# mims-harvard/Raindrop

Measured on AMD Instinct MI355X. Metric: samples/sec fwd+bwd, P19 34-sensor batch=256; % HBM roofline on msg-pass kernel, higher is better.
Workload: dtype f32

## Files before the change

### raindrop_amd/csrc/rd_attnfuse.hip

```cpp
#include <stdlib.h>

#include "rd_common.h"
#include "rd_plan.h"
#include "rd_rng.h"

namespace rd {
namespace {

typedef __bf16 bf8 __attribute__((ext_vector_type(8)));
typedef __bf16 bf4 __attribute__((ext_vector_type(4)));
typedef short sh4 __attribute__((ext_vector_type(4)));
typedef short sh8 __attribute__((ext_vector_type(8)));

constexpr int TS = 64;
constexpr int LDT = TS;
__device__ __forceinline__ int tsw(int row) { return (row & 3) | (((row >> 3) & 1) << 2); }
__device__ __forceinline__ int tofs(int row, int col) { return row * LDT + ((((col >> 3) ^ tsw(row)) & 7) << 3) + (col & 7); }
constexpr int AF_WV = 8, AF_THR = 64 * AF_WV;

struct FAttnArgs {
  const float* x;
  const __bf16* wf;
  const __bf16* wb;
  const float* bias;
  float* out; float* lse;
  const float* dout; const float* ds1; float* dx;
  __bf16* xt; __bf16* dt;
  const int32_t* plan;
  int T, B, D, H, hd;
  float scale, p_drop; uint64_t seed; uint32_t site; const uint64_t* seed_cell;
  int one;
  unsigned long long* stamps;
};
static unsigned long long* g_af_stamps = nullptr;
#define AFSTAMP(i)                                                                                  \
  do {                                                                                              \
    if (a.stamps && blockIdx.x == 0 && threadIdx.x == 0) a.stamps[(i)] = clock64();                 \
  } while (0)

__device__ __forceinline__ float g16_max(float v) {
#define RD_ROR(v, n) __builtin_bit_cast(float, __builtin_amdgcn_update_dpp(0, __builtin_bit_cast(int, v), 0x120 + (n), 0xf, 0xf, false))
  v = fmaxf(v, RD_ROR(v, 8)); v = fmaxf(v, RD_ROR(v, 4)); v = fmaxf(v, RD_ROR(v, 2)); v = fmaxf(v, RD_ROR(v, 1));
  return v;
}
__device__ __forceinline__ float g16_sum(float v) {
  v += RD_ROR(v, 8); v += RD_ROR(v, 4); v += RD_ROR(v, 2); v += RD_ROR(v, 1);
#undef RD_ROR
  return v;
}

__device__ __forceinline__ bf8 frag_n(const __bf16* P, int ld, int row0, int k0, int lane) {
  return *reinterpret_cast<const bf8*>(P + (row0 + (lane & 15)) * ld + k0 + 8 * (lane >> 4));
}
__device__ __forceinline__ bf8 frag_t(const __bf16* P, int ld, int k0, int col0, int lane) {
  const int i = lane & 15, G = lane >> 4;
  const __bf16* src = P + (k0 + 8 * G + (i >> 2)) * ld + col0 + 4 * (i & 3);
  const sh4 lo = __builtin_amdgcn_ds_read_tr16_b64_v4i16((sh4 __attribute__((address_space(3)))*)(src));
  const sh4 hi = __builtin_amdgcn_ds_read_tr16_b64_v4i16((sh4 __attribute__((address_space(3)))*)(src + 4 * ld));
  const sh8 o = {lo[0], lo[1], lo[2], lo[3], hi[0], hi[1], hi[2], hi[3]};
  return __builtin_bit_cast(bf8, o);
}
__device__ __forceinline__ bf8 frag_ns(const __bf16* P, int row0, int k0, int lane) {
  return *reinterpret_cast<const bf8*>(P + tofs(row0 + (lane & 15), k0 + 8 * (lane >> 4)));
}
__device__ __forceinline__ bf8 frag_ts(const __bf16* P, int k0, int col0, int lane) {
  const int i = lane & 15, G = lane >> 4;
  const int row = k0 + 8 * G + (i >> 2), col = col0 + 4 * (i & 3);
  const __bf16* src = P + tofs(row, col);
  const sh4 lo = __builtin_amdgcn_ds_read_tr16_b64_v4i16((sh4 __attribute__((address_space(3)))*)(src));
  const sh4 hi = __builtin_amdgcn_ds_read_tr16_b64_v4i16((sh4 __attribute__((address_space(3)))*)(src + 4 * LDT));
  const sh8 o = {lo[0], lo[1], lo[2], lo[3], hi[0], hi[1], hi[2], hi[3]};
  return __builtin_bit_cast(bf8, o);
}
template <int NT, bool AT, bool BT, bool ASW, bool BSW>
__device__ __forceinline__ void mma_b16(f32x4 (&acc)[NT], const __bf16* Ah, const __bf16* Al, int lda, int a0, const __bf16* Bh,
                                        const __bf16* Bl, int ldb, int b0, int KK, int lane, bool one) {
  auto fa = [&](const __bf16* P, int k0) {
    if (ASW) return AT ? frag_ts(P, k0, a0, lane) : frag_ns(P, a0, k0, lane);
    return AT ? frag_t(P, lda, k0, a0, lane) : frag_n(P, lda, a0, k0, lane);
  };
  auto fb = [&](const __bf16* P, int k0, int j) {
    if (BSW) return BT ? frag_ts(P, k0, b0 + 16 * j, lane) : frag_ns(P, b0 + 16 * j, k0, lane);
    return BT ? frag_t(P, ldb, k0, b0 + 16 * j, lane) : frag_n(P, ldb, b0 + 16 * j, k0, lane);
  };
  if (!one) {
#pragma unroll
    for (int k0 = 0; k0 < KK; k0 += 32) {
      const bf8 ah = fa(Ah, k0);
      const bf8 al = fa(Al, k0);
      bf8 bh[NT], bl[NT];
#pragma unroll
      for (int j = 0; j < NT; ++j) { bh[j] = fb(Bh, k0, j); bl[j] = fb(Bl, k0, j); }
#pragma unroll
      for (int j = 0; j < NT; ++j) acc[j] = __builtin_amdgcn_mfma_f32_16x16x32_bf16(al, bh[j], acc[j], 0, 0, 0);
#pragma unroll
      for (int j = 0; j < NT; ++j) acc[j] = __builtin_amdgcn_mfma_f32_16x16x32_bf16(ah, bl[j], acc[j], 0, 0, 0);
#pragma unroll
      for (int j = 0; j < NT; ++j) acc[j] = __builtin_amdgcn_mfma_f32_16x16x32_bf16(ah, bh[j], acc[j], 0, 0, 0);
    }
  } else {
#pragma unroll
    for (int k0 = 0; k0 < KK; k0 += 32) {
      const bf8 ah = fa(Ah, k0);
#pragma unroll
      for (int j = 0; j < NT; ++j) {
        const bf8 bh = fb(Bh, k0, j);
        acc[j] = __builtin_amdgcn_mfma_f32_16x16x32_bf16(ah, bh, acc[j], 0, 0, 0);
      }
    }
  }
}

__device__ __forceinline__ void split4(const float (&v)[4], bf4& hi, bf4& lo) {
#pragma unroll
  for (int r = 0; r < 4; ++r) { hi[r] = (__bf16)v[r]; lo[r] = (__bf16)(v[r] - (float)hi[r]); }
}
__device__ __forceinline__ void store_t4(__bf16* Ph, __bf16* Pl, int row, int col4, const float (&v)[4]) {
  bf4 hi, lo;
  split4(v, hi, lo);
  const int o = tofs(row, col4);
  *reinterpret_cast<bf4*>(Ph + o) = hi;
  *reinterpret_cast<bf4*>(Pl + o) = lo;
}

__device__ __forceinline__ uint64_t attn_quad(int bh, int T, int q, int key) { return ((uint64_t)bh * T + key) * ((T + 3) >> 2) + (q >> 2); }
__device__ __forceinline__ void attn_keep4(float (&k4)[4], uint64_t seed, uint32_t site, int bh, int T, int q0, int key, float p, float inv_keep) {
  const float4 u = uniform4(seed, site, attn_quad(bh, T, q0, key));
  k4[0] = u.x >= p ? inv_keep : 0.f; k4[1] = u.y >= p ? inv_keep : 0.f;
  k4[2] = u.z >= p ? inv_keep : 0.f; k4[3] = u.w >= p ? inv_keep : 0.f;
}

template <int KCX>
struct XRows { float4 v[(TS * 8 * KCX) / AF_THR]; };

template <int KCX>
__device__ __forceinline__ void x_request(XRows<KCX>& r, const float* x, long row0, int Tv, int D, int tid) {
  constexpr int kq = 8 * KCX, NIT = (TS * kq) / AF_THR;
  static_assert((TS * kq) % AF_THR == 0, "x tile must divide over the workgroup");
#pragma unroll
  for (int it = 0; it < NIT; ++it) {
    const int i = tid + it * AF_THR;
    const int rr = i / kq, k = 4 * (i - rr * kq);
    r.v[it] = *reinterpret_cast<const float4*>(x + (row0 + min(rr, Tv - 1)) * D + min(k, D - 4));
  }
}
template <int KCX>
__device__ __forceinline__ void x_store(const XRows<KCX>& r, __bf16* Xh, __bf16* Xl, int Tv, int D, int tid) {
  constexpr int kq = 8 * KCX, NIT = (TS * kq) / AF_THR, LDX = 32 * KCX + 16;
#pragma unroll
  for (int it = 0; it < NIT; ++it) {
    const int i = tid + it * AF_THR;
    const int rr = i / kq, k = 4 * (i - rr * kq);
    const bool ok = rr < Tv && k < D;
    const float v[4] = {ok ? r.v[it].x : 0.f, ok ? r.v[it].y : 0.f, ok ? r.v[it].z : 0.f, ok ? r.v[it].w : 0.f};
    bf4 hi, lo;
    split4(v, hi, lo);
    *reinterpret_cast<bf4*>(Xh + rr * LDX + k) = hi;
    *reinterpret_cast<bf4*>(Xl + rr * LDX + k) = lo;
  }
}

template <int KCX>
struct QkvPanel { bf8 h[2][KCX], l[2][KCX]; float bs[2]; };

template <int NTH, int KCX>
__device__ __forceinline__ void qkv_request(QkvPanel<KCX>& p, const __bf16* wf_h, const float* bias, int D, int hd, int h, int wave, int lane) {
  constexpr int NCT3 = 3 * NTH;
  static_assert(NCT3 <= 2 * AF_WV, "two column tiles per wave");
#pragma unroll
  for (int s = 0; s < 2; ++s) {
    const int ct = min(wave + AF_WV * s, NCT3 - 1);
    const __bf16* t = wf_h + (size_t)ct * (KCX * 2 * 512) + lane * 8;
#pragma unroll
    for (int kc = 0; kc < KCX; ++kc) {
      p.h[s][kc] = *reinterpret_cast<const bf8*>(t + (kc * 2 + 0) * 512);
      p.l[s][kc] = *reinterpret_cast<const bf8*>(t + (kc * 2 + 1) * 512);
    }
    const int whc = ct / NTH, cl = 16 * (ct - whc * NTH) + (lane & 15);
    p.bs[s] = bias[whc * D + h * hd + min(cl, hd - 1)];
  }
}

template <int NTH, int KCX>
__device__ __forceinline__ void qkv_project(const QkvPanel<KCX>& p, const __bf16* Xh, const __bf16* Xl, int hd, int Tv, __bf16* Tp, int wave,
                                            int lane, bool one) {
  constexpr int NCT3 = 3 * NTH, HDP = 32 * ((16 * NTH + 31) / 32), LDX = 32 * KCX + 16;
  const bool two = wave + AF_WV < NCT3;
  const int aoff = (lane & 15) * LDX + 8 * (lane >> 4);
  f32x4 acc[2][4];
#pragma unroll
  for (int s = 0; s < 2; ++s)
#pragma unroll
    for (int rt = 0; rt < 4; ++rt) acc[s][rt] = (f32x4){0.f, 0.f, 0.f, 0.f};
  if (!one) {
#pragma unroll
    for (int kc = 0; kc < KCX; ++kc) {
      bf8 ah[4], al[4];
#pragma unroll
      for (int rt = 0; rt < 4; ++rt) {
        ah[rt] = *reinterpret_cast<const bf8*>(Xh + rt * 16 * LDX + aoff + kc * 32);
        al[rt] = *reinterpret_cast<const bf8*>(Xl + rt * 16 * LDX + aoff + kc * 32);
      }
#pragma unroll
      for (int s = 0; s < 2; ++s)
#pragma unroll
        for (int rt = 0; rt < 4; ++rt) acc[s][rt] = __builtin_amdgcn_mfma_f32_16x16x32_bf16(al[rt], p.h[s][kc], acc[s][rt], 0, 0, 0);
#pragma unroll
      for (int s = 0; s < 2; ++s)
#pragma unroll
        for (int rt = 0; rt < 4; ++rt) acc[s][rt] = __builtin_amdgcn_mfma_f32_16x16x32_bf16(ah[rt], p.l[s][kc], acc[s][rt], 0, 0, 0);
#pragma unroll
      for (int s = 0; s < 2; ++s)
#pragma unroll
        for (int rt = 0; rt < 4; ++rt) acc[s][rt] = __builtin_amdgcn_mfma_f32_16x16x32_bf16(ah[rt], p.h[s][kc], acc[s][rt], 0, 0, 0);
    }
  } else {
#pragma unroll
    for (int kc = 0; kc < KCX; ++kc) {
#pragma unroll
      for (int rt = 0; rt < 4; ++rt) {
        const bf8 ah = *reinterpret_cast<const bf8*>(Xh + rt * 16 * LDX + aoff + kc * 32);
#pragma unroll
        for (int s = 0; s < 2; ++s) acc[s][rt] = __builtin_amdgcn_mfma_f32_16x16x32_bf16(ah, p.h[s][kc], acc[s][rt], 0, 0, 0);
      }
    }
  }
#pragma unroll
  for (int s = 0; s < 2; ++s) {
    if (s == 1 && !two) break;
    const int ct = wave + AF_WV * s;
    const int whc = ct / NTH, cl = 16 * (ct - whc * NTH) + (lane & 15);
    __bf16* Ph = Tp + (size_t)(whc * 2) * HDP * LDT;
    __bf16* Pl = Ph + (size_t)HDP * LDT;
    const bool cok = cl < hd;
#pragma unroll
    for (int rt = 0; rt < 4; ++rt) {
      const int r0 = 16 * rt + 4 * (lane >> 4);
      float v[4];
#pragma unroll
      for (int r = 0; r < 4; ++r) v[r] = (cok && r0 + r < Tv) ? acc[s][rt][r] + p.bs[s] : 0.f;
      store_t4(Ph, Pl, cl, r0, v);
    }
  }
}

template <int NTH>
__device__ __forceinline__ void zero_pad_rows(__bf16* Tp, int tid) {
  constexpr int HDP = 32 * ((16 * NTH + 31) / 32), PADR = HDP - 16 * NTH;
  if (PADR == 0) return;
  constexpr int Q8 = LDT / 4;
  for (int i = tid; i < 6 * PADR * Q8; i += AF_THR) {
    const int pl = i / (PADR * Q8), rem = i - pl * (PADR * Q8);
    const int rr = rem / Q8, q = rem - rr * Q8;
    bf4 z;
#pragma unroll
    for (int c = 0; c < 4; ++c) z[c] = (__bf16)0.f;
    *reinterpret_cast<bf4*>(Tp + ((size_t)pl * HDP + 16 * NTH + rr) * LDT + 4 * q) = z;
  }
}

template <int NTH, int KCX, bool ONE>
__global__ __launch_bounds__(AF_THR) void k_attn_fwd_fused(FAttnArgs a) {
  extern __shared__ __attribute__((aligned(16))) unsigned char fsm[];
  RD_TOUCH_CODE(ONE ? RD_TL_ATTN_FWD_B : RD_TL_ATTN_FWD);
  constexpr int HDP = 32 * ((16 * NTH + 31) / 32), LDX = 32 * KCX + 16, NA = (NTH + 1) / 2;
  constexpr int LDO = 16 * NTH + 4;
  __bf16* Xh = reinterpret_cast<__bf16*>(fsm);
  __bf16* Xl = Xh + TS * LDX;
  __bf16* Tp = Xl + TS * LDX;
  __bf16 *Qh = Tp, *Ql = Qh + HDP * LDT, *Kh = Ql + HDP * LDT, *Kl = Kh + HDP * LDT, *Vh = Kl + HDP * LDT, *Vl = Vh + HDP * LDT;
  float* mxs = reinterpret_cast<float*>(Vl + HDP * LDT);
  float* sms = mxs + 2 * TS;
  __bf16 *Ph = Qh, *Pl = Ql;
  float* ost = reinterpret_cast<float*>(Kh);
  static_assert(HDP >= TS, "P^T must fit inside the Q^T plane");
  static_assert((size_t)TS * LDO * 4 <= (size_t)2 * HDP * LDT * 2, "output stage must fit inside the K^T planes");
  const int tid = threadIdx.x, lane = tid & 63, wave = __builtin_amdgcn_readfirstlane(tid >> 6), wq = wave & 3, wh = wave >> 2;
  const int b = blockIdx.x;
  const int Tv = __builtin_amdgcn_readfirstlane(a.plan[plan::len_base(a.B) + b]);
  if (Tv <= 0) return;
  const long row0 = __builtin_amdgcn_readfirstlane(a.plan[plan::off_base() + b]);
  uint64_t seedv = a.seed;
  XRows<KCX> xr;
  x_request<KCX>(xr, a.x, row0, Tv, a.D, tid);
  QkvPanel<KCX> pan;
  qkv_request<NTH, KCX>(pan, a.wf, a.bias, a.D, a.hd, 0, wave, lane);
  __builtin_amdgcn_sched_barrier(0);
  if (a.p_drop > 0.f && a.seed_cell) seedv += load_uniform_u64(a.seed_cell);
  zero_pad_rows<NTH>(Tp, tid);
  AFSTAMP(0);
  x_store<KCX>(xr, Xh, Xl, Tv, a.D, tid);
  AFSTAMP(1);
  lds_barrier();
  AFSTAMP(2);
  const float inv_keep = 1.0f / (1.0f - a.p_drop);
  constexpr bool one = ONE;
  const int qr0 = wq * 16 + 4 * (lane >> 4);
  for (int h = 0; h < a.H; ++h) {
    const int bh = b * a.H + h;
    if (h > 0) zero_pad_rows<NTH>(Tp, tid);
    qkv_project<NTH, KCX>(pan, Xh, Xl, a.hd, Tv, Tp, wave, lane, one);
    __builtin_amdgcn_sched_barrier(0);
    {
      const int hn = h + 1 < a.H ? h + 1 : 0;
      qkv_request<NTH, KCX>(pan, a.wf + (size_t)hn * (3 * NTH * KCX * 2 * 512), a.bias, a.D, a.hd, hn, wave, lane);
    }
    __builtin_amdgcn_sched_barrier(0);
    AFSTAMP(3 + 8 * h);
    lds_barrier();
    AFSTAMP(4 + 8 * h);
    float kp[2][4];
#pragma unroll
    for (int j = 0; j < 2; ++j)
      attn_keep4(kp[j], seedv, a.site, bh, a.T, qr0, min(16 * (2 * wh + j) + (lane & 15), a.T - 1), a.p_drop, inv_keep);
    f32x4 s[2];
#pragma unroll
    for (int j = 0; j < 2; ++j) s[j] = (f32x4){0.f, 0.f, 0.f, 0.f};
    mma_b16<2, true, true, true, true>(s, Qh, Ql, LDT, wq * 16, Kh, Kl, LDT, 32 * wh, HDP, lane, one);
    float mx[4] = {-INFINITY, -INFINITY, -INFINITY, -INFINITY};
#pragma unroll
    for (int j = 0; j < 2; ++j) {
      const int key = 16 * (2 * wh + j) + (lane & 15);
      const bool dead = key >= Tv;
#pragma unroll
      for (int r = 0; r < 4; ++r) {
        s[j][r] = dead ? -INFINITY : s[j][r] * a.scale;
        mx[r] = fmaxf(mx[r], s[j][r]);
      }
    }
#pragma unroll
    for (int r = 0; r < 4; ++r) {
      mx[r] = g16_max(mx[r]);
      if ((lane & 15) == 0) mxs[wh * TS + qr0 + r] = mx[r];
    }
    AFSTAMP(5 + 8 * h);
    lds_barrier();
    float m_i[4], rsum[4] = {0.f, 0.f, 0.f, 0.f};
#pragma unroll
    for (int r = 0; r < 4; ++r) m_i[r] = fmaxf(mxs[qr0 + r], mxs[TS + qr0 + r]);
#pragma unroll
    for (int j = 0; j < 2; ++j) {
      const int key = 16 * (2 * wh + j) + (lane & 15);
      float pv[4];
#pragma unroll
      for (int r = 0; r < 4; ++r) {
        const float p = (s[j][r] == -INFINITY) ? 0.f : __expf(s[j][r] - m_i[r]);
        rsum[r] += p;
        pv[r] = p * kp[j][r];
      }
      store_t4(Ph, Pl, key, qr0, pv);
    }
#pragma unroll
    for (int r = 0; r < 4; ++r) {
      rsum[r] = g16_sum(rsum[r]);
      if ((lane & 15) == 0) sms[wh * TS + qr0 + r] = rsum[r];
    }
    AFSTAMP(6 + 8 * h);
    lds_barrier();
    AFSTAMP(7 + 8 * h);
    float l_i[4];
#pragma unroll
    for (int r = 0; r < 4; ++r) l_i[r] = sms[qr0 + r] + sms[TS + qr0 + r];
    const int t0 = wh * NA;
    f32x4 o[NA];
#pragma unroll
    for (int j = 0; j < NA; ++j) o[j] = (f32x4){0.f, 0.f, 0.f, 0.f};
    mma_b16<NA, true, false, true, true>(o, Ph, Pl, LDT, wq * 16, Vh, Vl, LDT, 16 * t0, TS, lane, one);
#pragma unroll
    for (int r = 0; r < 4; ++r) {
      const int q = qr0 + r;
      const float inv = 1.0f / l_i[r];
#pragma unroll
      for (int j = 0; j < NA; ++j)
        if (t0 + j < NTH) ost[q * LDO + 16 * (t0 + j) + (lane & 15)] = o[j][r] * inv;
      if (wh == 0 && (lane & 15) == 0 && q < Tv) a.lse[(long)bh * a.T + q] = m_i[r] + logf(l_i[r]);
    }
    AFSTAMP(8 + 8 * h);
    lds_barrier();
    AFSTAMP(9 + 8 * h);
    {
      const int qpr = a.hd >> 2;
      for (int e = tid; e < Tv * qpr; e += AF_THR) {
        const int q = e / qpr, c4 = e - q * qpr;
        *reinterpret_cast<float4*>(a.out + (row0 + q) * a.D + h * a.hd + 4 * c4) = *reinterpret_cast<const float4*>(ost + q * LDO + 4 * c4);
      }
    }
    lds_barrier();
    AFSTAMP(10 + 8 * h);
  }
}

template <int NTH, int KCX>
constexpr size_t fwd_lds() {
  constexpr int HDP = 32 * ((16 * NTH + 31) / 32), LDX = 32 * KCX + 16;
  return (size_t)2 * TS * LDX * 2 + (size_t)6 * HDP * LDT * 2 + (size_t)4 * TS * 4;
}

template <int NTH>
struct HRegs { float4 v[(4 * NTH + 7) / 8]; unsigned ok; };
template <int NTH>
__device__ __forceinline__ void head_request(HRegs<NTH>& h, const float* base, long ld, int Tv, int hd, int tl) {
  constexpr int NCH = (4 * NTH + 7) / 8;
  const int t = tl >> 3;
  const bool rok = t < Tv;
  const float* src = base + (long)(rok ? t : 0) * ld;
  unsigned ok = 0;
#pragma unroll
  for (int i = 0; i < NCH; ++i) {
    const int c = 4 * ((tl & 7) + 8 * i);
    const bool cok = c < hd;
    h.v[i] = *reinterpret_cast<const float4*>(src + (cok ? c : 0));
    if (rok && cok) ok |= 1u << i;
  }
  h.ok = ok;
}
template <int NTH>
__device__ __forceinline__ void head_mask(HRegs<NTH>& h) {
  constexpr int NCH = (4 * NTH + 7) / 8;
#pragma unroll
  for (int i = 0; i < NCH; ++i)
    if (!((h.ok >> i) & 1u)) h.v[i] = make_float4(0.f, 0.f, 0.f, 0.f);
}

template <int KB>
struct DxPanel { bf8 h[2][KB], l[2][KB]; };

template <int KCX, int KB, int NS>
__device__ __forceinline__ void dx_request(DxPanel<KB>& p, const __bf16* wb_h, int which, int wave, int lane) {
  constexpr int NCT = 2 * KCX;
#pragma unroll
  for (int s = 0; s < NS; ++s) {
    const __bf16* t = wb_h + ((size_t)which * NCT + wave + AF_WV * s) * (KB * 2 * 512) + lane * 8;
#pragma unroll
    for (int kc = 0; kc < KB; ++kc) {
      p.h[s][kc] = *reinterpret_cast<const bf8*>(t + (kc * 2 + 0) * 512);
      p.l[s][kc] = *reinterpret_cast<const bf8*>(t + (kc * 2 + 1) * 512);
    }
  }
}
template <int NTH, int KB, int NS, bool ONE>
__device__ __forceinline__ void dx_mma(f32x4 (&dxa)[2][4], const DxPanel<KB>& p, const __bf16* Tp, int which, int lane) {
  constexpr int HDP = 32 * ((16 * NTH + 31) / 32);
  const __bf16* Ah = Tp + (size_t)(which * 2) * HDP * LDT;
  const __bf16* Al = Ah + (size_t)HDP * LDT;
#pragma unroll
  for (int kc = 0; kc < KB; ++kc) {
    bf8 ah[4], al[4];
#pragma unroll
    for (int rt = 0; rt < 4; ++rt) {
      ah[rt] = frag_ts(Ah, 32 * kc, 16 * rt, lane);
      if (!ONE) al[rt] = frag_ts(Al, 32 * kc, 16 * rt, lane);
    }
    if (!ONE) {
#pragma unroll
      for (int s = 0; s < NS; ++s)
#pragma unroll
        for (int rt = 0; rt < 4; ++rt) dxa[s][rt] = __builtin_amdgcn_mfma_f32_16x16x32_bf16(al[rt], p.h[s][kc], dxa[s][rt], 0, 0, 0);
#pragma unroll
      for (int s = 0; s < NS; ++s)
#pragma unroll
        for (int rt = 0; rt < 4; ++rt) dxa[s][rt] = __builtin_amdgcn_mfma_f32_16x16x32_bf16(ah[rt], p.l[s][kc], dxa[s][rt], 0, 0, 0);
    }
#pragma unroll
    for (int s = 0; s < NS; ++s)
#pragma unroll
      for (int rt = 0; rt < 4; ++rt) dxa[s][rt] = __builtin_amdgcn_mfma_f32_16x16x32_bf16(ah[rt], p.h[s][kc], dxa[s][rt], 0, 0, 0);
  }
}
template <int NTH, int KCX, int NS, bool ONE>
__device__ __forceinline__ void dx_phase(f32x4 (&dxa)[2][4], DxPanel<(16 * NTH + 31) / 32>& p0, const __bf16* Tp, const __bf16* wb_h, int wave,
                                         int lane) {
  constexpr int KB = (16 * NTH + 31) / 32;
  DxPanel<KB> p1;
  dx_request<KCX, KB, NS>(p1, wb_h, 1, wave, lane);
  __builtin_amdgcn_sched_barrier(0);
  dx_mma<NTH, KB, NS, ONE>(dxa, p0, Tp, 0, lane);
  __builtin_amdgcn_sched_barrier(0);
  dx_request<KCX, KB, NS>(p0, wb_h, 2, wave, lane);
  __builtin_amdgcn_sched_barrier(0);
  dx_mma<NTH, KB, NS, ONE>(dxa, p1, Tp, 1, lane);
  __builtin_amdgcn_sched_barrier(0);
  dx_mma<NTH, KB, NS, ONE>(dxa, p0, Tp, 2, lane);
  __builtin_amdgcn_sched_barrier(0);
}

template <int NTH, int KCX, bool ONE>
__global__ __launch_bounds__(AF_THR) void k_attn_bwd_fused(FAttnArgs a) {
  extern __shared__ __attribute__((aligned(16))) unsigned char fsm[];
  RD_TOUCH_CODE(ONE ? RD_TL_ATTN_BWD_B : RD_TL_ATTN_BWD);
  constexpr int HDP = 32 * ((16 * NTH + 31) / 32), LDX = 32 * KCX + 16, NA = (NTH + 1) / 2, KB = HDP / 32, LDB = HDP + 16;
  constexpr int NCT = 2 * KCX;
  constexpr int LDS_DX = 32 * KCX + 4;
  __bf16* Xh = reinterpret_cast<__bf16*>(fsm);
  __bf16* Xl = Xh + TS * LDX;
  __bf16 *Ph = Xh, *Pl = Ph + TS * LDT, *Sh = Pl + TS * LDT, *Sl = Sh + TS * LDT;
  float* dxs = reinterpret_cast<float*>(fsm);
  static_assert((size_t)4 * TS * LDT * 2 <= (size_t)2 * TS * LDX * 2, "score planes must fit inside the x planes");
  static_assert((size_t)TS * LDS_DX * 4 <= (size_t)2 * TS * LDX * 2, "dx stage must fit inside the x planes");
  __bf16* Tp = Xl + TS * LDX;
  __bf16 *Qh = Tp, *Ql = Qh + HDP * LDT, *Kh = Ql + HDP * LDT, *Kl = Kh + HDP * LDT, *Vh = Kl + HDP * LDT, *Vl = Vh + HDP * LDT;
  __bf16* Oh = Vl + HDP * LDT;
  __bf16* Ol = Oh + TS * LDB;
  float* lse_s = reinterpret_cast<float*>(Ol + TS * LDB);
  float* dl_s = lse_s + TS;
  const int tid = threadIdx.x, lane = tid & 63, wave = __builtin_amdgcn_readfirstlane(tid >> 6), wq = wave & 3, wh = wave >> 2;
  const int b = blockIdx.x;
  const int Tv = __builtin_amdgcn_readfirstlane(a.plan[plan::len_base(a.B) + b]);
  if (Tv <= 0) return;
  const long row0 = __builtin_amdgcn_readfirstlane(a.plan[plan::off_base() + b]);
  const int g0 = __builtin_amdgcn_readfirstlane(a.plan[plan::coff_base(a.B, a.T) + b]);
  const int ngrp = (Tv + 15) >> 4;
  const bool tail_zero = (g0 + ngrp) == __builtin_amdgcn_readfirstlane(a.plan[plan::coff_base(a.B, a.T) + a.B]) && ((g0 + ngrp) & 1);
  uint64_t seedv = a.seed;
  if (a.p_drop > 0.f && a.seed_cell) seedv += load_uniform_u64(a.seed_cell);
  const float inv_keep = 1.0f / (1.0f - a.p_drop);
  constexpr bool one = ONE;
  f32x4 dxa[2][4];
#pragma unroll
  for (int s = 0; s < 2; ++s)
#pragma unroll
    for (int rt = 0; rt < 4; ++rt) dxa[s][rt] = (f32x4){0.f, 0.f, 0.f, 0.f};
  const bool two = wave + AF_WV < NCT;
  constexpr int NQ = (TS * 8 * KCX + AF_THR - 1) / AF_THR;
  QkvPanel<KCX> pan;
  HRegs<NTH> dov, ov; float lrow;
  head_request<NTH>(dov, a.dout + row0 * a.D, a.D, Tv, a.hd, tid);
  head_request<NTH>(ov, a.out + row0 * a.D, a.D, Tv, a.hd, tid);
  lrow = a.lse[(long)(b * a.H) * a.T + min(tid >> 3, Tv - 1)];
  for (int h = 0; h < a.H; ++h) {
    const int bh = b * a.H + h;
    int tl = tid;
    asm volatile("" : "+v"(tl));
    XRows<KCX> xr;
    x_request<KCX>(xr, a.x, row0, Tv, a.D, tl);
    int lq = lane;
    asm volatile("" : "+v"(lq));
    qkv_request<NTH, KCX>(pan, a.wf + (size_t)h * (3 * NTH * KCX * 2 * 512), a.bias, a.D, a.hd, h, wave, lq);
    AFSTAMP(32 + 16 * h);
    __builtin_amdgcn_sched_barrier(0);
    if (h == 0) zero_pad_rows<NTH>(Tp, tl);
    x_store<KCX>(xr, Xh, Xl, Tv, a.D, tl);
    AFSTAMP(33 + 16 * h);
    lds_barrier();
    AFSTAMP(34 + 16 * h);
    if (h == 0) {
      const int i16 = lq & 15, g2 = (lq >> 4) & 1, sub = lq >> 5;
      const int npair = (ngrp + 1) >> 1;
      for (int t = wave; t < npair * NCT * 2; t += AF_WV) {
        const int plane = t & 1, cj = t >> 1;
        const int pr = cj / NCT, j = cj - pr * NCT;
        const int lg = 2 * pr + sub;
        const __bf16* src = (plane ? Xl : Xh) + (16 * min(lg, ngrp - 1) + 8 * g2 + (i16 >> 2)) * LDX + 16 * j + 4 * (i16 & 3);
        const sh4 lo = __builtin_amdgcn_ds_read_tr16_b64_v4i16((sh4 __attribute__((address_space(3)))*)(src));
        const sh4 hi = __builtin_amdgcn_ds_read_tr16_b64_v4i16((sh4 __attribute__((address_space(3)))*)(src + 4 * LDX));
        const sh8 o = {lo[0], lo[1], lo[2], lo[3], hi[0], hi[1], hi[2], hi[3]};
        const int gg = g0 + lg;
        if (lg < ngrp)
          *reinterpret_cast<sh8*>(a.xt + (((size_t)(gg >> 1) * NCT + j) * 2 + plane) * 512 + (32 * (gg & 1) + 16 * g2 + i16) * 8) = o;
      }
      if (tail_zero) {
        const int gg = g0 + ngrp;
        const sh8 z = {0, 0, 0, 0, 0, 0, 0, 0};
        for (int i = tid; i < NCT * 2 * 32; i += AF_THR) {
          const int slot = i & 31, jp = i >> 5;
          *reinterpret_cast<sh8*>(a.xt + ((size_t)(gg >> 1) * NCT * 2 + jp) * 512 + (32 + slot) * 8) = z;
        }
      }
    }
    {
      constexpr int NCH = (4 * NTH + 7) / 8;
      head_mask<NTH>(dov);
      head_mask<NTH>(ov);
      float d = 0.f;
#pragma unroll
      for (int i = 0; i < NCH; ++i)
        d += (dov.v[i].x * ov.v[i].x + dov.v[i].y * ov.v[i].y) + (dov.v[i].z * ov.v[i].z + dov.v[i].w * ov.v[i].w);
      d += __shfl_xor(d, 1);
      d += __shfl_xor(d, 2);
      d += __shfl_xor(d, 4);
      const int o = (tl >> 3) * LDB + 4 * (tl & 7);
#pragma unroll
      for (int i = 0; i < NCH; ++i) {
        static_assert(32 * NCH == HDP, "8 threads x NCH chunks cover exactly the padded head width (chunks >= hd arrive as zeros)");
        const float v[4] = {dov.v[i].x, dov.v[i].y, dov.v[i].z, dov.v[i].w};
        bf4 hi, lo;
        split4(v, hi, lo);
        *reinterpret_cast<bf4*>(Oh + o + 32 * i) = hi;
        *reinterpret_cast<bf4*>(Ol + o + 32 * i) = lo;
      }
      if ((tl & 7) == 0) { dl_s[tl >> 3] = d; lse_s[tl >> 3] = lrow; }
    }
    __builtin_amdgcn_sched_barrier(0);
    {
      const int hn = h + 1 < a.H ? h + 1 : 0;
      head_request<NTH>(dov, a.dout + row0 * a.D + hn * a.hd, a.D, Tv, a.hd, tl);
      head_request<NTH>(ov, a.out + row0 * a.D + hn * a.hd, a.D, Tv, a.hd, tl);
      lrow = a.lse[(long)(b * a.H + hn) * a.T + min(tl >> 3, Tv - 1)];
    }
    AFSTAMP(35 + 16 * h);
    __builtin_amdgcn_sched_barrier(0);
    qkv_project<NTH, KCX>(pan, Xh, Xl, a.hd, Tv, Tp, wave, lq, one);
    AFSTAMP(36 + 16 * h);
    lds_barrier();
    AFSTAMP(37 + 16 * h);
    int l1 = lane;
    asm volatile("" : "+v"(l1));
    const int qr1 = wq * 16 + 4 * (l1 >> 4);
    float kp[2][4];
#pragma unroll
    for (int j = 0; j < 2; ++j)
      attn_keep4(kp[j], seedv, a.site, bh, a.T, qr1, min(16 * (2 * wh + j) + (l1 & 15), a.T - 1), a.p_drop, inv_keep);
    f32x4 s[2], dp[2];
#pragma unroll
    for (int j = 0; j < 2; ++j) { s[j] = (f32x4){0.f, 0.f, 0.f, 0.f}; dp[j] = s[j]; }
    mma_b16<2, true, true, true, true>(s, Qh, Ql, LDT, wq * 16, Kh, Kl, LDT, 32 * wh, HDP, l1, one);
    mma_b16<2, false, true, false, true>(dp, Oh, Ol, LDB, wq * 16, Vh, Vl, LDT, 32 * wh, HDP, l1, one);
#pragma unroll
    for (int j = 0; j < 2; ++j) {
      const int key = 16 * (2 * wh + j) + (l1 & 15);
      const bool dead = key >= Tv;
      const float (&k4)[4] = kp[j];
      float pm[4], ds[4];
#pragma unroll
      for (int r = 0; r < 4; ++r) {
        const int row = qr1 + r;
        pm[r] = 0.f; ds[r] = 0.f;
        if (!dead && row < Tv) {
          const float p = __expf(s[j][r] * a.scale - lse_s[row]);
          pm[r] = p * k4[r];
          ds[r] = p * (dp[j][r] * k4[r] - dl_s[row]) * a.scale;
        }
      }
      store_t4(Ph, Pl, key, qr1, pm);
      store_t4(Sh, Sl, key, qr1, ds);
    }
    AFSTAMP(38 + 16 * h);
    lds_barrier();
    AFSTAMP(39 + 16 * h);
    const int t0 = wh * NA;
    int l2 = lane;
    asm volatile("" : "+v"(l2));
    f32x4 dq[NA], dk[NA], dv[NA];
#pragma unroll
    for (int j = 0; j < NA; ++j) { dq[j] = (f32x4){0.f, 0.f, 0.f, 0.f}; dk[j] = dq[j]; dv[j] = dq[j]; }
    mma_b16<NA, true, false, true, true>(dq, Sh, Sl, LDT, wq * 16, Kh, Kl, LDT, 16 * t0, TS, l2, one);
    mma_b16<NA, false, false, true, true>(dk, Sh, Sl, LDT, wq * 16, Qh, Ql, LDT, 16 * t0, TS, l2, one);
    mma_b16<NA, false, true, true, false>(dv, Ph, Pl, LDT, wq * 16, Oh, Ol, LDB, 16 * t0, TS, l2, one);
    AFSTAMP(40 + 16 * h);
    lds_barrier();
    AFSTAMP(41 + 16 * h);
    const __bf16* wb_h = a.wb + (size_t)h * (3 * NCT * KB * 2 * 512);
    DxPanel<KB> dp0;
    int ld = lane;
    asm volatile("" : "+v"(ld));
    if (two) dx_request<KCX, KB, 2>(dp0, wb_h, 0, wave, ld); else dx_request<KCX, KB, 1>(dp0, wb_h, 0, wave, ld);
    __builtin_amdgcn_sched_barrier(0);
#pragma unroll
    for (int j = 0; j < NA; ++j) {
      if (t0 + j < NTH) {
        const int f = 16 * (t0 + j) + (ld & 15), qr2 = wq * 16 + 4 * (ld >> 4);
        const float vq[4] = {dq[j][0], dq[j][1], dq[j][2], dq[j][3]};
        const float vk[4] = {dk[j][0], dk[j][1], dk[j][2], dk[j][3]};
        const float vv[4] = {dv[j][0], dv[j][1], dv[j][2], dv[j][3]};
        store_t4(Qh, Ql, f, qr2, vq);
        store_t4(Kh, Kl, f, qr2, vk);
        store_t4(Vh, Vl, f, qr2, vv);
      }
    }
    AFSTAMP(42 + 16 * h);
    lds_barrier();
    AFSTAMP(43 + 16 * h);
    {
      const int i16 = ld & 15, g2 = (ld >> 4) & 1, sub = ld >> 5;
      const int nctp = 3 * a.H * NTH;
      const int npair = (ngrp + 1) >> 1;
      for (int t = wave; t < 3 * NTH * npair * 2; t += AF_WV) {
        const int plane = t & 1, u = t >> 1;
        const int pr = u / (3 * NTH), wj = u - pr * (3 * NTH);
        const int which = wj / NTH, j = wj - which * NTH;
        const int lg = 2 * pr + sub;
        const __bf16* src = Tp + (size_t)(which * 2 + plane) * HDP * LDT + tofs(16 * j + i16, 16 * min(lg, ngrp - 1) + 8 * g2);
        const sh8 o = *reinterpret_cast<const sh8*>(src);
        const int jt = (which * a.H + h) * NTH + j;
        const int gg = g0 + lg;
        if (lg < ngrp)
          *reinterpret_cast<sh8*>(a.dt + (((size_t)(gg >> 1) * nctp + jt) * 2 + plane) * 512 + (32 * (gg & 1) + 16 * g2 + i16) * 8) = o;
      }
      if (tail_zero) {
        const int gg = g0 + ngrp;
        const sh8 z = {0, 0, 0, 0, 0, 0, 0, 0};
        for (int i = tid; i < 3 * NTH * 2 * 32; i += AF_THR) {
          const int slot = i & 31, jp = i >> 5;
          const int wj = jp >> 1, plane = jp & 1;
          const int which = wj / NTH, j = wj - which * NTH;
          const int jt = (which * a.H + h) * NTH + j;
          *reinterpret_cast<sh8*>(a.dt + (((size_t)(gg >> 1) * nctp + jt) * 2 + plane) * 512 + (32 + slot) * 8) = z;
        }
      }
    }
    AFSTAMP(44 + 16 * h);
    if (two) { if (one) dx_phase<NTH, KCX, 2, true>(dxa, dp0, Tp, wb_h, wave, ld); else dx_phase<NTH, KCX, 2, false>(dxa, dp0, Tp, wb_h, wave, ld); }
    else { if (one) dx_phase<NTH, KCX, 1, true>(dxa, dp0, Tp, wb_h, wave, ld); else dx_phase<NTH, KCX, 1, false>(dxa, dp0, Tp, wb_h, wave, ld); }
    AFSTAMP(45 + 16 * h);
  }
  float4 r4[NQ];
  {
    const int qpr = a.D >> 2;
#pragma unroll
    for (int i = 0; i < NQ; ++i) {
      const int e = tid + i * AF_THR, q = e / qpr, c4 = e - q * qpr;
      r4[i] = *reinterpret_cast<const float4*>(a.ds1 + (row0 + min(q, Tv - 1)) * a.D + 4 * c4);
    }
  }
  __builtin_amdgcn_sched_barrier(0);
#pragma unroll
  for (int s = 0; s < 2; ++s) {
    if (s == 1 && !two) break;
    const int ct = wave + AF_WV * s;
#pragma unroll
    for (int rt = 0; rt < 4; ++rt)
#pragma unroll
      for (int r = 0; r < 4; ++r) dxs[(16 * rt + 4 * (lane >> 4) + r) * LDS_DX + 16 * ct + (lane & 15)] = dxa[s][rt][r];
  }
  AFSTAMP(64);
  lds_barrier();
  {
    const int qpr = a.D >> 2;
#pragma unroll
    for (int i = 0; i < NQ; ++i) {
      const int e = tid + i * AF_THR, q = e / qpr, c4 = e - q * qpr;
      if (q < Tv) {
        const float4 s4 = *reinterpret_cast<const float4*>(dxs + q * LDS_DX + 4 * c4);
        *reinterpret_cast<float4*>(a.dx + (row0 + q) * a.D + 4 * c4) = make_float4(s4.x + r4[i].x, s4.y + r4[i].y, s4.z + r4[i].z, s4.w + r4[i].w);
      }
    }
  }
  AFSTAMP(65);
}

template <int NTH, int KCX>
constexpr size_t bwd_lds() {
  constexpr int HDP = 32 * ((16 * NTH + 31) / 32), LDX = 32 * KCX + 16, LDB = HDP + 16;
  return (size_t)2 * TS * LDX * 2 + (size_t)6 * HDP * LDT * 2 + (size_t)2 * TS * LDB * 2 + (size_t)2 * TS * 4;
}

constexpr int AF_NTH = 5, AF_KCX = 5;

}

extern "C" void rd_debug_set_attnfuse_stamps(void* p) { g_af_stamps = (unsigned long long*)p; }

bool attnfuse_ok(int T, int D, int H, int hd) {
  const char* e = getenv("RD_ATTN_FUSE");
  const bool enabled = !(e && atoi(e) == 0);
  return enabled && precision() != RD_PREC_FP32 && T <= TS && hd <= 16 * AF_NTH && hd * H == D && (D + 31) / 32 == AF_KCX && (D % 4) == 0 &&
         (hd % 4) == 0 && H >= 1 && H <= 2 && 3 * AF_NTH <= 2 * AF_WV;
}
size_t attnfuse_wf_elems(int H) { return (size_t)H * 3 * AF_NTH * AF_KCX * 2 * 512; }
size_t attnfuse_wb_elems(int H) { return (size_t)H * 3 * (2 * AF_KCX) * ((16 * AF_NTH + 31) / 32) * 2 * 512; }
int attnfuse_split_specs(const float* in_proj_w, int D, int H, int hd, void* wf, void* wb, WsplitSpec* out) {
  constexpr int KB = (16 * AF_NTH + 31) / 32;
  int n = 0;
  for (int h = 0; h < H; ++h)
    for (int which = 0; which < 3; ++which) {
      const float* W = in_proj_w + ((size_t)which * D + (size_t)h * hd) * D;
      out[n++] = WsplitSpec{W, hd, D, 0, (__bf16*)wf + ((size_t)(h * 3 + which) * AF_NTH) * (AF_KCX * 2 * 512)};
      out[n++] = WsplitSpec{W, hd, D, 1, (__bf16*)wb + ((size_t)(h * 3 + which) * (2 * AF_KCX)) * (KB * 2 * 512)};
    }
  return n;
}
int attnfuse_padded_cols(int H) { return 3 * H * 16 * AF_NTH; }
int attnfuse_nth() { return AF_NTH; }

static void fill_args(FAttnArgs& a, const float* x, const void* wf, const void* wb, const float* bias, const int32_t* plan, int T, int B,
                      int D, int H, int hd, float p_drop, uint64_t seed, uint32_t site) {
  a.x = x; a.wf = (const __bf16*)wf; a.wb = (const __bf16*)wb; a.bias = bias; a.plan = plan;
  a.T = T; a.B = B; a.D = D; a.H = H; a.hd = hd;
  a.scale = 1.0f / sqrtf((float)hd); a.p_drop = p_drop; a.seed = seed; a.site = site; a.seed_cell = seed_cell();
  a.one = precision() == RD_PREC_BF16; a.stamps = g_af_stamps;
}

int launch_attn_fused_fwd(const float* x, const void* wf, const float* bias, const int32_t* plan, int T, int B, int D, int H, int hd,
                          float p_drop, uint64_t seed, uint32_t site, float* out, float* lse, hipStream_t st) {
  if (!plan) return fail(RD_EINVAL, "fused attention: needs a token plan");
  FAttnArgs a{};
  fill_args(a, x, wf, nullptr, bias, plan, T, B, D, H, hd, p_drop, seed, site);
  a.out = out; a.lse = lse;
  constexpr size_t lds = fwd_lds<AF_NTH, AF_KCX>();
  if (a.one) { RD_LDS_ATTR((k_attn_fwd_fused<AF_NTH, AF_KCX, true>), lds);
               hipLaunchKernelGGL((k_attn_fwd_fused<AF_NTH, AF_KCX, true>), dim3(B), dim3(AF_THR), lds, st, a); }
  else { RD_LDS_ATTR((k_attn_fwd_fused<AF_NTH, AF_KCX, false>), lds);
         hipLaunchKernelGGL((k_attn_fwd_fused<AF_NTH, AF_KCX, false>), dim3(B), dim3(AF_THR), lds, st, a); }
  return check_launch("k_attn_fwd_fused");
}

int launch_attn_fused_bwd(const float* x, const void* wf, const void* wb, const float* bias, const int32_t* plan, int T, int B, int D, int H,
                          int hd, float p_drop, uint64_t seed, uint32_t site, const float* out, const float* lse, const float* dout,
                          const float* ds1, float* dx, void* xt, void* dt, hipStream_t st) {
  if (!plan) return fail(RD_EINVAL, "fused attention: needs a token plan");
  FAttnArgs a{};
  fill_args(a, x, wf, wb, bias, plan, T, B, D, H, hd, p_drop, seed, site);
  a.out = const_cast<float*>(out); a.lse = const_cast<float*>(lse); a.dout = dout; a.ds1 = ds1; a.dx = dx;
  a.xt = (__bf16*)xt; a.dt = (__bf16*)dt;
  constexpr size_t lds = bwd_lds<AF_NTH, AF_KCX>();
  if (a.one) { RD_LDS_ATTR((k_attn_bwd_fused<AF_NTH, AF_KCX, true>), lds);
               hipLaunchKernelGGL((k_attn_bwd_fused<AF_NTH, AF_KCX, true>), dim3(B), dim3(AF_THR), lds, st, a); }
  else { RD_LDS_ATTR((k_attn_bwd_fused<AF_NTH, AF_KCX, false>), lds);
         hipLaunchKernelGGL((k_attn_bwd_fused<AF_NTH, AF_KCX, false>), dim3(B), dim3(AF_THR), lds, st, a); }
  return check_launch("k_attn_bwd_fused");
}

}
```

### raindrop_amd/csrc/rd_touch_gen.h

```cpp
#pragma once
#define RD_TL_K1_FWD_P19 13056
#define RD_TL_K1_BWD_P19 10368
#define RD_TL_K1_FWD 16640
#define RD_TL_K1_BWD 11648
#define RD_TL_ATTN_FWD 12800
#define RD_TL_ATTN_BWD 26368
#define RD_TL_ATTN_FWD_B 11136
#define RD_TL_ATTN_BWD_B 19968
#define RD_TL_EF_POST_P19L 41856
#define RD_TL_EF_POST_P19L_B 38272
#define RD_TL_EF_POST_P19 41472
#define RD_TL_EF_POST_P19_B 37888
#define RD_TL_EF_POST_P12L 41344
#define RD_TL_EF_POST_P12L_B 37760
#define RD_TL_EF_POST_P12 40960
#define RD_TL_EF_POST_P12_B 37376
#define RD_TL_EF_POST_RTL 53376
#define RD_TL_EF_POST_RTL_B 49792
#define RD_TL_EF_POST_RT 56320
#define RD_TL_EF_POST_RT_B 52736
#define RD_TL_EF_PRE_P19L 43776
#define RD_TL_EF_PRE_P19L_B 40320
#define RD_TL_EF_PRE_P19 43392
#define RD_TL_EF_PRE_P19_B 39936
#define RD_TL_EF_PRE_P12L 43264
#define RD_TL_EF_PRE_P12L_B 39936
#define RD_TL_EF_PRE_P12 42880
#define RD_TL_EF_PRE_P12_B 39552
#define RD_TL_EF_PRE_RTL 59648
#define RD_TL_EF_PRE_RTL_B 55936
#define RD_TL_EF_PRE_RT 59264
#define RD_TL_EF_PRE_RT_B 55552
#define RD_TL_DW 7424
#define RD_TL_DW_REDUCE 9984
#define RD_TL_ADAM 2944
#define RD_TL_ADAM_DEV 3072
#define RD_TL_WSPLIT 5248
#define RD_TL_TWG 10496
#define RD_TL_TWG_ONE 8832
#define RD_TL_HEAD_P19 15616
#define RD_TL_HEAD 17152
#define RD_TL_GEMM 26368
#define RD_TL_GEMM_X3 30080
#define RD_TL_GEMM_PANEL 33024
#define RD_TL_GEMM_PANEL_WIDE 111232
#define RD_TL_GEMM_PANEL_PC 55552
#define RD_TL_ROWGEMM 4480
#define RD_TL_ATTN_FWD_ONE 6144
#define RD_TL_ATTN_BWD_ONE 6528
#define RD_TL_ATTN_FWD_B16 7424
#define RD_TL_ATTN_BWD_DQ 7552
#define RD_TL_ATTN_BWD_DKV 6400
#define RD_TL_ADD_LN_FWD 5632
#define RD_TL_LN_BWD_R 5632
#define RD_TL_LN_BWD_V 6656
```

Baseline: 760,200.

## Prefetch next head's X rows and QKV weights during attention backward

Restructures the per-head loop in the fused attention backward kernel so the X-row load and the QKV weight-panel load for head h+1 are issued inside head h, overlapping the dK/dV MMAs and the dx phase. The first head's loads move into a prologue before the loop. The dx phase is moved ahead of the transposed-gradient store so the weight request can follow it. This hides global-load latency at the top of each head iteration, at the cost of longer live register ranges and possible register pressure. It also issues a dummy weight load on the last head.

Result: slower. 751,200 (-1.2%).

```diff
diff --git a/raindrop_amd/csrc/rd_attnfuse.hip b/raindrop_amd/csrc/rd_attnfuse.hip
--- a/raindrop_amd/csrc/rd_attnfuse.hip
+++ b/raindrop_amd/csrc/rd_attnfuse.hip
@@ -164,13 +164,14 @@
 struct QkvPanel { bf8 h[2][KCX], l[2][KCX]; float bs[2]; };
 
 template <int NTH, int KCX>
-__device__ __forceinline__ void qkv_request(QkvPanel<KCX>& p, const __bf16* wf_h, const float* bias, int D, int hd, int h, int wave, int lane) {
+__device__ __forceinline__ void qkv_request(QkvPanel<KCX>& p, const __bf16* wf_h, const float* bias, int D, int hd, int h, int wave, int lane,
+                                            bool live = true) {
   constexpr int NCT3 = 3 * NTH;
   static_assert(NCT3 <= 2 * AF_WV, "two column tiles per wave");
 #pragma unroll
   for (int s = 0; s < 2; ++s) {
     const int ct = min(wave + AF_WV * s, NCT3 - 1);
-    const __bf16* t = wf_h + (size_t)ct * (KCX * 2 * 512) + lane * 8;
+    const __bf16* t = wf_h + (size_t)ct * (KCX * 2 * 512) + lane * (live ? 8 : 0);
 #pragma unroll
     for (int kc = 0; kc < KCX; ++kc) {
       p.h[s][kc] = *reinterpret_cast<const bf8*>(t + (kc * 2 + 0) * 512);
@@ -527,20 +528,26 @@
   head_request<NTH>(dov, a.dout + row0 * a.D, a.D, Tv, a.hd, tid);
   head_request<NTH>(ov, a.out + row0 * a.D, a.D, Tv, a.hd, tid);
   lrow = a.lse[(long)(b * a.H) * a.T + min(tid >> 3, Tv - 1)];
+  {
+    int tp = tid, lp = lane;
+    asm volatile("" : "+v"(tp));
+    asm volatile("" : "+v"(lp));
+    XRows<KCX> xr;
+    x_request<KCX>(xr, a.x, row0, Tv, a.D, tp);
+    qkv_request<NTH, KCX>(pan, a.wf, a.bias, a.D, a.hd, 0, wave, lp);
+    AFSTAMP(32);
+    __builtin_amdgcn_sched_barrier(0);
+    zero_pad_rows<NTH>(Tp, tp);
+    x_store<KCX>(xr, Xh, Xl, Tv, a.D, tp);
+    AFSTAMP(33);
+  }
   for (int h = 0; h < a.H; ++h) {
     const int bh = b * a.H + h;
+    const bool more = h + 1 < a.H;
     int tl = tid;
     asm volatile("" : "+v"(tl));
-    XRows<KCX> xr;
-    x_request<KCX>(xr, a.x, row0, Tv, a.D, tl);
     int lq = lane;
     asm volatile("" : "+v"(lq));
-    qkv_request<NTH, KCX>(pan, a.wf + (size_t)h * (3 * NTH * KCX * 2 * 512), a.bias, a.D, a.hd, h, wave, lq);
-    AFSTAMP(32 + 16 * h);
-    __builtin_amdgcn_sched_barrier(0);
-    if (h == 0) zero_pad_rows<NTH>(Tp, tl);
-    x_store<KCX>(xr, Xh, Xl, Tv, a.D, tl);
-    AFSTAMP(33 + 16 * h);
     lds_barrier();
     AFSTAMP(34 + 16 * h);
     if (h == 0) {
@@ -637,6 +644,9 @@
     AFSTAMP(38 + 16 * h);
     lds_barrier();
     AFSTAMP(39 + 16 * h);
+    XRows<KCX> xr;
+    if (more) x_request<KCX>(xr, a.x, row0, Tv, a.D, tl);
+    __builtin_amdgcn_sched_barrier(0);
     const int t0 = wh * NA;
     int l2 = lane;
     asm volatile("" : "+v"(l2));
@@ -668,8 +678,19 @@
       }
     }
     AFSTAMP(42 + 16 * h);
+    if (more) x_store<KCX>(xr, Xh, Xl, Tv, a.D, tl);
+    AFSTAMP(46 + 16 * h);
     lds_barrier();
     AFSTAMP(43 + 16 * h);
+    if (two) { if (one) dx_phase<NTH, KCX, 2, true>(dxa, dp0, Tp, wb_h, wave, ld); else dx_phase<NTH, KCX, 2, false>(dxa, dp0, Tp, wb_h, wave, ld); }
+    else { if (one) dx_phase<NTH, KCX, 1, true>(dxa, dp0, Tp, wb_h, wave, ld); else dx_phase<NTH, KCX, 1, false>(dxa, dp0, Tp, wb_h, wave, ld); }
+    AFSTAMP(45 + 16 * h);
+    {
+      const int hn = more ? h + 1 : 0;
+      qkv_request<NTH, KCX>(pan, a.wf + (size_t)hn * (3 * NTH * KCX * 2 * 512), a.bias, a.D, a.hd, hn, wave, ld, more);
+    }
+    AFSTAMP(47 + 16 * h);
+    __builtin_amdgcn_sched_barrier(0);
     {
       const int i16 = ld & 15, g2 = (ld >> 4) & 1, sub = ld >> 5;
       const int nctp = 3 * a.H * NTH;
@@ -699,9 +720,6 @@
       }
     }
     AFSTAMP(44 + 16 * h);
-    if (two) { if (one) dx_phase<NTH, KCX, 2, true>(dxa, dp0, Tp, wb_h, wave, ld); else dx_phase<NTH, KCX, 2, false>(dxa, dp0, Tp, wb_h, wave, ld); }
-    else { if (one) dx_phase<NTH, KCX, 1, true>(dxa, dp0, Tp, wb_h, wave, ld); else dx_phase<NTH, KCX, 1, false>(dxa, dp0, Tp, wb_h, wave, ld); }
-    AFSTAMP(45 + 16 * h);
   }
   float4 r4[NQ];
   {
diff --git a/raindrop_amd/csrc/rd_touch_gen.h b/raindrop_amd/csrc/rd_touch_gen.h
--- a/raindrop_amd/csrc/rd_touch_gen.h
+++ b/raindrop_amd/csrc/rd_touch_gen.h
@@ -4,9 +4,9 @@
 #define RD_TL_K1_FWD 16640
 #define RD_TL_K1_BWD 11648
 #define RD_TL_ATTN_FWD 12800
-#define RD_TL_ATTN_BWD 26368
+#define RD_TL_ATTN_BWD 28544
 #define RD_TL_ATTN_FWD_B 11136
-#define RD_TL_ATTN_BWD_B 19968
+#define RD_TL_ATTN_BWD_B 22144
 #define RD_TL_EF_POST_P19L 41856
 #define RD_TL_EF_POST_P19L_B 38272
 #define RD_TL_EF_POST_P19 41472
```
